# DassHydro-dev/smash

Measured on AMD Instinct MI355X. Metric: cell-timesteps/s, forward+adjoint sweep, higher is better.
Workload: dtype f32

## Files before the change

### __graft_entry__.py

```python
from __future__ import annotations

import os
import subprocess
import sys

ROOT = os.path.dirname(os.path.abspath(__file__))
if ROOT not in sys.path:
    sys.path.insert(0, ROOT)

HIPCC = os.environ.get("HIPCC", "/opt/rocm/bin/hipcc")
CSRC = os.path.join(ROOT, "smash_amd", "csrc")
LIB = os.path.join(ROOT, "smash_amd", "libsmashx.so")
LIB_EXACT = os.path.join(ROOT, "smash_amd", "libsmashx_exact.so")
HIP_FLAGS = ["-O3", "-ffp-contract=off", "--offload-arch=gfx950", "-fPIC", "-shared", "-std=c++17"]


def _newer(target, sources):
    if not os.path.exists(target):
        return False
    t = os.path.getmtime(target)
    return all(os.path.getmtime(s) <= t for s in sources)


def build() -> None:
    srcs = [os.path.join(CSRC, f) for f in sorted(os.listdir(CSRC)) if f.endswith((".hip", ".cpp", ".h"))]
    srcs += [os.path.join(ROOT, "include", "smashx.h"), os.path.join(ROOT, "include", "smashx_setup.h"),
             os.path.join(ROOT, "include", "smashx_forcing.h"), os.path.join(ROOT, "include", "smashx_prcp.h"),
             os.path.join(ROOT, "include", "smashx_signature.h"), os.path.join(ROOT, "include", "smashx_hyper.h"),
             os.path.join(ROOT, "include", "smashx_ann.h")]
    jobs = []
    for lib, extra in ((LIB, []), (LIB_EXACT, ["-DSX_EXACT_LIBM=1"])):
        if not _newer(lib, srcs):
            cmd = [HIPCC] + HIP_FLAGS + extra + ["-pthread", "-o", lib, os.path.join(CSRC, "smashx.hip"), os.path.join(CSRC, "sx_plan.cpp"),
                                                 os.path.join(CSRC, "sx_lbfgsb.cpp"), os.path.join(CSRC, "sx_hyper.cpp")]
            jobs.append((cmd, subprocess.Popen(cmd, cwd=ROOT)))
    for cmd, j in jobs:
        if j.wait() != 0:
            raise subprocess.CalledProcessError(j.returncode, cmd)
    subprocess.check_call(["make", "-s", "-C", os.path.join(ROOT, "oracle"), "liboracle.so", "liboracle64.so"])
    ref_src = os.environ.get("SMASH_REFERENCE", "/root/reference")
    ref_lib = os.path.join(ROOT, "oracle", "_ref", "libsmash_ref.so")
    dropin = os.path.join(ROOT, "oracle", "_ref", "libsmash_dropin.so")
    shim = [os.path.join(ROOT, "fortran", "smashx_dropin.f90"), os.path.join(ROOT, "fortran", "smashx_setulb.f90"),
            os.path.join(ROOT, "include", "smashx.h"), os.path.join(ROOT, "oracle", "ref", "ref_capi.f90"),
            os.path.join(ROOT, "oracle", "ref", "build_ref.sh")]
    native_lb = os.path.join(ROOT, "oracle", "_ref", "libsmash_dropin_lbfgsb.so")
    if os.path.isdir(os.path.join(ref_src, "smash", "solver")) and not (os.path.exists(ref_lib) and _newer(dropin, shim) and _newer(native_lb, shim)):
        subprocess.check_call(["bash", os.path.join(ROOT, "oracle", "ref", "build_ref.sh")])
    import smash_amd
    from smash_amd import _lib
    L = _lib.lib()
    missing = [s for s in _lib.SYMBOLS + _lib.SETUP_SYMBOLS + _lib.FORCING_SYMBOLS + _lib.PRCP_SYMBOLS + _lib.SIGNATURE_SYMBOLS + _lib.HYPER_DEVICE_SYMBOLS + _lib.ANN_SYMBOLS if not hasattr(L, s)]
    if missing:
        raise RuntimeError(f"libsmashx.so lacks {missing}")


def smoke() -> None:
    import numpy as np

    sys.path.insert(0, os.path.join(ROOT, "tests"))
    import golden_util as gu

    import smash_amd
    from oracle import pyoracle
    if not os.path.exists(LIB):
        build()
    g = gu.load("gr_b_16x16x96_nse_gaps")
    ref = pyoracle.run(g.structure, g.mesh, g.dt, g.prcp, g.pet, g.qobs, g.params, g.states, adjoint=True, **g.opts)
    for k, v in g.adj["parameters_b"].items():
        assert np.array_equal(ref["parameters_b"][k], v), k

    setup = smash_amd.SetupDT(0, g.mesh.ng, structure=g.structure, dt=g.dt, ntime_step=g.nt)
    setup.optimize.jobs_fun, setup.optimize.wjobs_fun = ["nse"], [1.0]
    mesh = smash_amd.MeshDT.from_synth(setup, g.mesh)
    inp = smash_amd.Input_DataDT(setup, mesh)
# ... 25 lines not shown
```

### include/smashx.h

```cpp
#ifndef SMASHX_H
#define SMASHX_H

#ifdef __cplusplus
extern "C" {
#endif

#define SMASHX_GNP 16
#define SMASHX_GNS 8

enum { SMASHX_GR_A = 1, SMASHX_GR_B = 2, SMASHX_GR_C = 3, SMASHX_GR_D = 4, SMASHX_VIC_A = 5 };
enum { SMASHX_NSE = 1, SMASHX_KGE = 2, SMASHX_KGE2 = 3, SMASHX_SE = 4, SMASHX_RMSE = 5, SMASHX_LOGARITHMIC = 6,
       SMASHX_CRC = 7, SMASHX_CFP2 = 8, SMASHX_CFP10 = 9, SMASHX_CFP50 = 10, SMASHX_CFP90 = 11, SMASHX_EPF = 12, SMASHX_ELT = 13,
       SMASHX_ERC = 14 };
enum { SMASHX_PRIOR = 1, SMASHX_SMOOTHING = 2, SMASHX_HARD_SMOOTHING = 3 };
enum { SMASHX_P_CI = 0, SMASHX_P_CP = 1, SMASHX_P_BETA = 2, SMASHX_P_CFT = 3, SMASHX_P_CST = 4, SMASHX_P_ALPHA = 5,
       SMASHX_P_EXC = 6, SMASHX_P_B = 7, SMASHX_P_CUSL1 = 8, SMASHX_P_CUSL2 = 9, SMASHX_P_CLSL = 10, SMASHX_P_KS = 11,
       SMASHX_P_DS = 12, SMASHX_P_DSM = 13, SMASHX_P_WS = 14, SMASHX_P_LR = 15 };
enum { SMASHX_S_HI = 0, SMASHX_S_HP = 1, SMASHX_S_HFT = 2, SMASHX_S_HST = 3, SMASHX_S_HUSL1 = 4, SMASHX_S_HUSL2 = 5,
       SMASHX_S_HLSL = 6, SMASHX_S_HLR = 7 };

enum {
    SMASHX_OK = 0,
    SMASHX_E_ARG = -1,
    SMASHX_E_UNSUPPORTED = -2,
// ... 186 lines not shown
};
int smashx_selftest_eval(int device, int fn, const float* x, const float* y, long long n, float* out0, float* out1);

#define SMASHX_LBFGSB_START 0
#define SMASHX_LBFGSB_FG 1
#define SMASHX_LBFGSB_NEW_X 2
#define SMASHX_LBFGSB_CONVERGED 3
#define SMASHX_LBFGSB_ABNORMAL 4
typedef struct smashx_lbfgsb smashx_lbfgsb;
int smashx_lbfgsb_create(long n, int m, const double* lower, const double* upper, double factr, double pgtol, smashx_lbfgsb** out);
int smashx_lbfgsb_step(smashx_lbfgsb* opt, double* x, double f, const double* g, int* task);
long smashx_lbfgsb_iterations(const smashx_lbfgsb* opt);
long smashx_lbfgsb_evaluations(const smashx_lbfgsb* opt);
double smashx_lbfgsb_projected_gradient(const smashx_lbfgsb* opt);
const char* smashx_lbfgsb_message(const smashx_lbfgsb* opt);
int smashx_lbfgsb_destroy(smashx_lbfgsb* opt);

#include "smashx_setup.h"
#include "smashx_forcing.h"
#include "smashx_prcp.h"
#include "smashx_signature.h"
#include "smashx_hyper.h"
#include "smashx_ann.h"

#ifdef __cplusplus
}
#endif
#endif
```

### smash_amd/_lib.py

```python
from __future__ import annotations

import ctypes as C
import os

_HERE = os.path.dirname(os.path.abspath(__file__))
EXACT = os.environ.get("SMASHX_EXACT_LIBM", "0") not in ("", "0")
LIB_PATH = os.environ.get("SMASHX_LIB", os.path.join(_HERE, "libsmashx_exact.so" if EXACT else "libsmashx.so"))

ABI_VERSION = 9
GNP, GNS = 16, 8
E_OK, E_ARG, E_UNSUPPORTED, E_HIP, E_NODEVICE, E_MESH, E_STATE = 0, -1, -2, -3, -4, -5, -6
STRUCTURES = {"gr-a": 1, "gr-b": 2, "gr-c": 3, "gr-d": 4, "vic-a": 5}
JOBS_FUN = {"nse": 1, "kge": 2, "kge2": 3, "se": 4, "rmse": 5, "logarithmic": 6,
            "Crc": 7, "Cfp2": 8, "Cfp10": 9, "Cfp50": 10, "Cfp90": 11, "Epf": 12, "Elt": 13, "Erc": 14}
SIGNATURE_FUN = ("Crc", "Cfp2", "Cfp10", "Cfp50", "Cfp90", "Epf", "Elt", "Erc")
JREG_FUN = {"prior": 1, "smoothing": 2, "hard_smoothing": 3}
HYPER = {"hyper-linear": 1, "hyper-polynomial": 2}
LBFGSB_START, LBFGSB_FG, LBFGSB_NEW_X, LBFGSB_CONVERGED, LBFGSB_ABNORMAL = range(5)
COMM_ID_BYTES = 128
FN = {k: i for i, k in enumerate("TANH TANH_BRANCHY EXPM1 EXP LOG POW POWB POW_M4 POW_M4_M5 POW_M025 POW_M025_M125 POW_3P5 POW_3P5_2P5 "
                                 "DIV DIV4 FDIV DIV_FAST".split())}
FN_COUNT = len(FN)

HALO_FN = C.CFUNCTYPE(C.c_int, C.c_void_p, C.c_int, C.c_int, C.c_int)
# ... 140 lines not shown
    "smashx_hyper_upload": (_int, [ptr, ptr, ptr]),
    "smashx_hyper_gradient": (_int, [ptr, ptr, ptr]),
    "smashx_hyper_fields": (_int, [ptr, _par, _sta]),
    "smashx_hyper_info": (_int, [ptr, ptr, ptr]),
}
HYPER_DEVICE_SYMBOLS = list(HYPER_DEVICE_PROTOTYPES)
ANN_LAYER = {"dense": 1, "relu": 2, "leaky_relu": 3, "elu": 4, "selu": 5, "sigmoid": 6, "tanh": 7, "scale": 8,
             "softplus": 9, "softmax": 10, "dropout": 11}
_graph = [_int, _int, ptr, ptr, _int]
ANN_PROTOTYPES = {
    "smashx_ann_set_descriptors": (_int, [ptr, _int, ptr]),
    "smashx_ann_set_net": (_int, [ptr, _int, ptr, ptr, _int, ptr, ptr, ptr]),
    "smashx_ann_upload": (_int, [ptr, ptr]),
    "smashx_ann_gradient": (_int, [ptr, ptr]),
    "smashx_ann_fields": (_int, [ptr, _par, _sta]),
    "smashx_ann_info": (_int, [ptr, ptr, ptr]),
    "smashx_ann_host_nweights": (_int, _graph),
    "smashx_ann_host_forward": (_int, _graph + [ptr, ptr, ptr, _long, ptr, ptr]),
    "smashx_ann_host_gradient": (_int, _graph + [ptr, ptr, ptr, _long, ptr, ptr, ptr]),
    "smashx_ann_host_activation": (_int, [_int, _long, ptr, ptr, ptr]),
    "smashx_ann_host_exp": (_int, [_long, ptr, ptr]),
}
ANN_SYMBOLS = list(ANN_PROTOTYPES)


class SmashxError(RuntimeError):
    def __init__(self, code, msg):
        super().__init__(f"libsmashx error {code}: {msg}")
        self.code = code


_lib = None


def lib():
    global _lib
    if _lib is None:
        if not os.path.exists(LIB_PATH):
            raise ImportError(f"{LIB_PATH} is missing: build the HIP library first (__graft_entry__.build()); "
                              "smash_amd has no CPU fallback")
        L = C.CDLL(LIB_PATH)
        for name, (restype, argtypes) in list(PROTOTYPES.items()) + list(SETUP_PROTOTYPES.items()) + list(FORCING_PROTOTYPES.items()) + list(PRCP_PROTOTYPES.items()) + list(SIGNATURE_PROTOTYPES.items()) + list(HYPER_DEVICE_PROTOTYPES.items()) + list(ANN_PROTOTYPES.items()):
            fn = getattr(L, name)
            fn.restype, fn.argtypes = restype, argtypes
        sizes = (C.c_int * 7)()
        L.smashx_abi_sizes(sizes)
        mine = [C.sizeof(t) for t in (Config, Mesh, Options, Parameters, States, Costs, Timing)]
        if list(sizes) != mine:
            raise ImportError(f"{LIB_PATH} was built from another include/smashx.h (struct sizes {list(sizes)}, this module expects {mine}): "
                              "rebuild it (__graft_entry__.build())")
        _lib = L
    return _lib


def check(rc):
    if rc != 0:
        raise SmashxError(rc, lib().smashx_last_error().decode())
```

### smash_amd/csrc/smashx.hip

```cpp
#include "../../include/smashx.h"

#include <hip/hip_runtime.h>
#include <rccl/rccl.h>

#include <dlfcn.h>

#include <algorithm>
#include <functional>
#include <numeric>
#include <cstdio>
#include <cstdlib>
#include <cstring>
#include <string>
#include <vector>

#include "sx_cost.h"
#include "sx_jreg.h"
#include "sx_kernels.h"
#include "sx_ensemble.h"
#include "sx_fields.h"
#include "sx_interception.h"
#include "sx_meanforcing.h"
#include "sx_prcpindices.h"
#include "sx_hypermap.h"
// ... 588 lines not shown
}

SxDeviceArrays view_at(const smashx_plan* p, int off) {
    SxDeviceArrays B = p->A;
    B.k0 = 0; B.k1 = p->n;
    const size_t q = (size_t)(off / 4);
    B.qtT = p->A.qtT + q * p->npad * 4;
    B.hrk = nullptr;
    if (p->A.hrT) { if (p->A.hr_skew) B.hr_row0 = (int)q; else B.hrT = p->A.hrT + q * p->npad * 4; }
    if (p->A.qdT) B.qdT = p->A.qdT + q * p->npad * 4;
    if (!p->chain) B.qsk = nullptr;
    B.xT = p->A.xT + q * p->A.nx * 4;
    if (p->A.qtdT) B.qtdT = p->A.qtdT + q * p->npad * 4;
    if (p->A.xdT) B.xdT = p->A.xdT + q * p->A.nx * 4;
    if (p->A.tape_hp) B.tape_hp = p->A.tape_hp + (size_t)off * p->npad;
    if (p->A.tape_hft) B.tape_hft = p->A.tape_hft + (size_t)off * p->npad;
    if (p->A.tape_hi) B.tape_hi = p->A.tape_hi + (size_t)off * p->npad;
    if (p->A.ckpt_hi) B.ckpt_hi = p->A.ckpt_hi + (size_t)(off / SX_HIK) * p->npad;
    if (p->A.tape_hst) B.tape_hst = p->A.tape_hst + (size_t)off * p->npad;
    return B;
}

typedef void (*VertKernel)(SxDeviceArrays, int, int);
VertKernel vert_fwd_kernel(int st, bool tape, bool compact) {
#define SX_GR(ST) {sx_k_vert_fwd<ST, false, false>, sx_k_vert_fwd<ST, false, true>, sx_k_vert_fwd<ST, true, false>, sx_k_vert_fwd<ST, true, true>}
    static const VertKernel k[5][4] = {SX_GR(1), SX_GR(2), SX_GR(3), SX_GR(4),
                                       {sx_k_vert_fwd_vic<false, false>, sx_k_vert_fwd_vic<false, true>, sx_k_vert_fwd_vic<true, false>, sx_k_vert_fwd_vic<true, true>}};
#undef SX_GR
    return k[st - 1][2 * tape + compact];
}
VertKernel vert_adj_kernel(int st, bool compact) {
    static const VertKernel k[5][2] = {{sx_k_vert_adj<1, false>, sx_k_vert_adj<1, true>}, {sx_k_vert_adj<2, false>, sx_k_vert_adj<2, true>},
                                       {sx_k_vert_adj<3, false>, sx_k_vert_adj<3, true>}, {sx_k_vert_adj<4, false>, sx_k_vert_adj<4, true>},
                                       {sx_k_vert_adj_vic<false>, sx_k_vert_adj_vic<true>}};
    return k[st - 1][compact];
}
VertKernel vert_tan_kernel(int st) {
    static const VertKernel k[5] = {sx_k_vert_fwd_d<1>, sx_k_vert_fwd_d<2>, sx_k_vert_fwd_d<3>, sx_k_vert_fwd_d<4>, sx_k_vert_fwd_vic_d};
    return k[st - 1];
}
void launch_vert(smashx_plan* p, VertKernel k, int kind, size_t lds, int off, int t0, int T) {
    const SxDeviceArrays B = view_at(p, off);
    if (B.k1 <= B.k0) return;
    const dim3 grid((B.k1 - B.k0 + SX_VBLOCK - 1) / SX_VBLOCK), block(SX_VBLOCK);
    p->mark_begin(kind, p->stream, (double)(B.k1 - B.k0) * T);
    hipLaunchKernelGGL(k, grid, block, lds, p->stream, B, t0, T);
    p->mark_end();
}
void vert_fwd(smashx_plan* p, int off, bool tape, int t0, int T) {
    launch_vert(p, vert_fwd_kernel(p->st, tape, p->A.prcp16 != nullptr), 0, p->st == 5 ? 0 : p->vlds_fwd, off, t0, T);
}
void vert_adj(smashx_plan* p, int off, int t0, int T) {
    launch_vert(p, vert_adj_kernel(p->st, p->A.prcp16 != nullptr), 3, p->st == 5 ? 0 : p->vlds_adj, off, t0, T);
}
void vert_tan(smashx_plan* p, int off, int t0, int T) { launch_vert(p, vert_tan_kernel(p->st), 0, 0, off, t0, T); }
double round_cells(const smashx_plan* p, int r0, int r1) {
    double c = 0.0;
    for (int r = r0; r < r1; ++r) c += p->round_ncells[r];
    return c;
}
int chain_first(const smashx_plan* p) {
    const int nr = p->sch.nrounds;
    return (p->chain && nr - p->chain_from >= 2) ? p->chain_from : nr;
}
void reset_chain_counters(smashx_plan* p, hipStream_t st) {
    (void)hipMemsetAsync(p->A.prog, 0, (size_t)p->sch.ngroups * sizeof(int), st);
    (void)hipMemsetAsync(p->A.prog + p->sch.ngroups + 1, 0, sizeof(int), st);
}
void route_fwd_rounds(smashx_plan* p, int off, bool tape, int t0, int T, hipStream_t st, int r0, int r1, int tan = 0) {
    SxDeviceArrays B = view_at(p, off);
    if (!p->dom_q_active) B.qdT = nullptr;
    if (tan) B.qsk = nullptr;
    const size_t lds = (size_t)2 * p->M * sizeof(float4);
    void (*const k)(SxDeviceArrays, int, int, int, int) = tan == 1 ? sx_k_route_fwd<true, false, 1> : tan == 2 ? sx_k_route_fwd<false, false, 2>
                                                         : tape ? sx_k_route_fwd<true, false> : sx_k_route_fwd<false, false>;
    for (int r = r0; r < r1; ++r) {
// ... 1351 lines not shown

int smashx_halo_edges(const smashx_plan* p, int* out_src, int* out_dst, int* in_src, int* in_dst) {
    if (!p) return fail(SMASHX_E_ARG, "null plan");
    for (int i = 0; i < p->n_out; ++i) { if (out_src) out_src[i] = p->sch.out_src[i]; if (out_dst) out_dst[i] = p->sch.out_dst[i]; }
    for (int i = 0; i < p->n_in; ++i) { if (in_src) in_src[i] = p->sch.in_src[i]; if (in_dst) in_dst[i] = p->sch.in_dst[i]; }
    return 0;
}

int smashx_plan_chunking(smashx_plan* p, int* chunk_steps, int* pipe_steps) {
    if (!p) return fail(SMASHX_E_ARG, "null plan");
    int rc = set_device(p); if (rc) return rc;
    if ((rc = ensure_chunk_buffers(p, true))) return rc;
    if (chunk_steps) *chunk_steps = p->Tc;
    if (pipe_steps) *pipe_steps = p->Tp;
    return 0;
}

int smashx_plan_hbm(const smashx_plan* p, double out[3]) {
    if (!p || !out) return fail(SMASHX_E_ARG, "null argument");
    out[0] = p->hbm_free_at_plan; out[1] = p->hbm_total; out[2] = p->bytes;
    return 0;
}

int smashx_set_halo(smashx_plan* p, float* d_out_buf, float* d_in_buf, smashx_halo_fn fn, void* user) {
    if (!p) return fail(SMASHX_E_ARG, "null plan");
    if (fn && ((p->n_out > 0 && !d_out_buf) || (p->n_in > 0 && !d_in_buf))) return fail(SMASHX_E_ARG, "halo buffers missing");
    p->halo_out = d_out_buf; p->halo_in = d_in_buf; p->halo_fn = fn; p->halo_user = user;
    return 0;
}

int smashx_set_median_slots(smashx_plan* p, int nslots, const int* slot_of_gauge, smashx_reduce_fn fn, void* user) {
    if (!p || nslots < 0 || (nslots > 0 && !slot_of_gauge)) return fail(SMASHX_E_ARG, "bad argument");
    int rc = set_device(p); if (rc) return rc;
    p->med_nslots = 0; p->med_fn = fn; p->med_user = user;
    if (nslots == 0) return 0;
    std::vector<int> sl(std::max(p->ng, 1), -1);
    for (int g = 0; g < p->ng; ++g) {
        sl[g] = slot_of_gauge[g];
        if (sl[g] < -1 || sl[g] >= nslots) return fail(SMASHX_E_ARG, "slot_of_gauge out of range");
    }
    if (p->d_med_slot) { p->dfree(p->d_med_slot); p->dfree(p->d_medx); p->dfree(p->d_medx_idx); }
    if ((rc = p->upload_vec(&p->d_med_slot, sl))) return rc;
    p->med_slot_h = sl;
    if ((rc = p->dmalloc(&p->d_medx, (size_t)3 * nslots))) return rc;
    if ((rc = p->dmalloc(&p->d_medx_idx, (size_t)nslots))) return rc;
    p->med_nslots = nslots;
// ... 1325 lines not shown
```

### smash_amd/csrc/sx_kernels.h

```cpp
#pragma once

#include <hip/hip_runtime.h>

#include <climits>

#include "sx_ops.h"
#include "sx_tangent.h"
#include "sx_vic.h"

#define SX_BT 4
#define SX_VBLOCK 256

__device__ __forceinline__ void sx_lds_barrier() {
    __builtin_amdgcn_fence(__ATOMIC_RELEASE, "workgroup", "local");
    __builtin_amdgcn_s_barrier();
    __builtin_amdgcn_fence(__ATOMIC_ACQUIRE, "workgroup", "local");
}

__device__ __forceinline__ void sx_lds_wave_fence() {
    __builtin_amdgcn_fence(__ATOMIC_RELEASE, "workgroup", "local");
    __builtin_amdgcn_wave_barrier();
    __builtin_amdgcn_fence(__ATOMIC_ACQUIRE, "workgroup", "local");
}

// ... 35 lines not shown
}
__device__ __forceinline__ void sx_gstore4(float4* p, const float4& q) {
#if defined(__HIP_DEVICE_COMPILE__)
    sx_f4v v; v.x = q.x; v.y = q.y; v.z = q.z; v.w = q.w;
    *(__attribute__((address_space(1))) sx_f4v*)p = v;
#else
    *p = q;
#endif
}
__device__ __forceinline__ float sx_gload1(const float* p) {
#if defined(__HIP_DEVICE_COMPILE__)
    return *(const __attribute__((address_space(1))) float*)p;
#else
    return *p;
#endif
}

__device__ __forceinline__ void sx_pin(float4& v) {
    asm volatile("" : "+v"(v.x), "+v"(v.y), "+v"(v.z), "+v"(v.w) : : "memory");
}

__device__ __forceinline__ void sx_pin1(float& v) { asm volatile("" : "+v"(v) : : "memory"); }
__device__ __forceinline__ void sx_pinu(unsigned& v) { asm volatile("" : "+v"(v) : : "memory"); }

typedef __attribute__((address_space(1))) int sx_gint;
#define SX_PROG_STALL(A) ((A).prog + (A).ngroups)
#define SX_PROG_TICKET(A) ((A).prog + (A).ngroups + 1)
#define SX_PROG_EXTRA 8
#ifndef SX_PK
#define SX_PK 16
#endif
#define SX_SPIN_LIMIT (1 << 22)
__device__ __forceinline__ void sx_wait_prog(const int* prog, int need, int& seen, int* stalled, int limit, int tag = -1) {
    if (seen >= need) return;
    int spins = 0;
    while (seen < need) {
        seen = __hip_atomic_load((const sx_gint*)prog, __ATOMIC_RELAXED, __HIP_MEMORY_SCOPE_AGENT);
        if (seen < need) {
            const bool out = ++spins > limit;
            if (out || (spins & 1023) == 0) {
                if (out) {
                    if (atomicCAS(stalled + 3, 0, tag + 2) == 0) { stalled[4] = (int)(prog - stalled); stalled[5] = need; stalled[6] = seen; }
                    __hip_atomic_store((sx_gint*)stalled, 1, __ATOMIC_RELAXED, __HIP_MEMORY_SCOPE_AGENT);
                }
                if (out || __hip_atomic_load((const sx_gint*)stalled, __ATOMIC_RELAXED, __HIP_MEMORY_SCOPE_AGENT)) { seen = 0x7fffffff; break; }
            }
// ... 136 lines not shown
    typedef int sx_v4i __attribute__((ext_vector_type(4)));
    const __amdgpu_buffer_rsrc_t r = __builtin_amdgcn_make_buffer_rsrc((void*)row, 0, 0x7fffffff, 0x00020000);
    sx_v4i v = {__builtin_bit_cast(int, a), __builtin_bit_cast(int, b), __builtin_bit_cast(int, c), __builtin_bit_cast(int, d)};
    __builtin_amdgcn_raw_buffer_store_b128(v, r, byte_off, 0, AUX);
}
template <int AUX = 0>
__device__ __forceinline__ void sx_row_store(float* row, unsigned byte_off, float v) {
    const __amdgpu_buffer_rsrc_t r = __builtin_amdgcn_make_buffer_rsrc((void*)row, 0, 0x7fffffff, 0x00020000);
    __builtin_amdgcn_raw_buffer_store_b32(__builtin_bit_cast(int, v), r, byte_off, 0, AUX);
}

template <int AUX = 0>
__device__ __forceinline__ unsigned sx_row_load_u16(const unsigned short* row, unsigned byte_off) {
    const __amdgpu_buffer_rsrc_t r = __builtin_amdgcn_make_buffer_rsrc((void*)row, 0, 0x7fffffff, 0x00020000);
    return (unsigned)(unsigned short)__builtin_amdgcn_raw_buffer_load_b16(r, byte_off, 0, AUX);
}

__device__ __forceinline__ float sx_prcp_decode(const SxDeviceArrays& A, unsigned k) {
    const float v = (float)k * A.prcp_c;
    return k == 65535u ? A.prcp_gap : v;
}

typedef const __attribute__((address_space(4))) float sx_cfloat;
template <bool COMPACT>
struct SxForcing {
    const SxDeviceArrays& A;
    const unsigned kb;
    const size_t npad;
    int h;
    const char* prow; const char* erow;
    unsigned p_n, p_w; float e_n, e_w, r_n, r_w;
    __device__ __forceinline__ SxForcing(const SxDeviceArrays& A_, unsigned kb_, int t_first)
        : A(A_), kb(kb_), npad((size_t)A_.npad), h(COMPACT ? (t_first + A_.hour0) % 24 : 0),
          prow(COMPACT ? (const char*)(A_.prcp16 + (size_t)t_first * A_.npad) : (const char*)(A_.prcp + (size_t)t_first * A_.npad)),
          erow(COMPACT ? nullptr : (const char*)(A_.pet + (size_t)t_first * A_.npad)),
          p_n(0u), p_w(0u), e_n(0.f), e_w(0.f), r_n(0.f), r_w(0.f) {}
    template <int AUX, bool BACK> __device__ __forceinline__ void request(int t, bool first) {
        const long step = (long)npad * (COMPACT ? 2 : 4) * (BACK ? -1 : 1);
        if (!COMPACT) {
            p_n = __float_as_uint(sx_row_load<AUX>((const float*)prow, kb));
            e_n = sx_row_load<AUX>((const float*)erow, kb);
            prow += step; erow += step;
            return;
        }
        p_n = __float_as_uint(sx_row_load<AUX>((const float*)prow, (kb >> 1) & ~3u));
        prow += step;
        if (first || h == (BACK ? 23 : 0)) e_n = sx_row_load<AUX>(A.petd + (size_t)((t + A.hour0) / 24) * npad, kb);
        r_n = sx_row_load(A.pet_ratio + h, 0u);
        h = BACK ? (h == 0 ? 23 : h - 1) : (h == 23 ? 0 : h + 1);
    }
    __device__ __forceinline__ void hold() {
        p_w = p_n; e_w = e_n; r_w = r_n;
        sx_pinu(p_w); sx_pin1(e_w);
        if (COMPACT) sx_pin1(r_w);
    }
    __device__ __forceinline__ float prcp() const {
        if (!COMPACT) return __uint_as_float(p_w);
        return sx_prcp_decode(A, (p_w >> ((kb & 4u) << 2)) & 0xffffu);
    }
    __device__ __forceinline__ float pet() const {
        if (!COMPACT) return e_w;
        return e_w < 0.f ? e_w : e_w * r_w;
    }
};

__device__ __forceinline__ void sx_forcing_at(const SxDeviceArrays& A, int t, unsigned kb, float& p, float& e) {
    const size_t npad = (size_t)A.npad;
    if (A.prcp16 == nullptr) { p = sx_row_load(A.prcp + (size_t)t * npad, kb); e = sx_row_load(A.pet + (size_t)t * npad, kb); return; }
    p = sx_prcp_decode(A, sx_row_load_u16(A.prcp16 + (size_t)t * npad, kb >> 1));
    const int q = t + A.hour0;
    const float D = sx_row_load(A.petd + (size_t)(q / 24) * npad, kb);
    e = D < 0.f ? D : D * ((sx_cfloat*)A.pet_ratio)[q % 24];
}

#ifndef SX_VFWD_WAVES
#define SX_VFWD_WAVES 8
#endif
template <int ST, bool TAPE, bool CF>
#ifndef SX_VFWD_WAVES_GRC
#define SX_VFWD_WAVES_GRC 7
#endif
__global__ __launch_bounds__(SX_VBLOCK, (ST == 2 && CF) ? SX_VFWD_WAVES : (ST == 3 && TAPE && CF) ? SX_VFWD_WAVES_GRC : 1)
void sx_k_vert_fwd(SxDeviceArrays A, int t0, int T) {
    SX_LIBM_INIT();
    const int k = A.k0 + blockIdx.x * SX_VBLOCK + threadIdx.x;
    if (k >= A.k1) return;
    const size_t npad = (size_t)A.npad;

    SxCellParams P;
    float hi = 0.f, hp = 0.f, hft = 0.f, hst = 0.f;
    P.ci = (ST == 2 || ST == 3) ? A.ci[k] : 1.f;
    P.cp = A.cp[k];
    P.cft = A.cft[k];
    P.cst = (ST == 3) ? A.cst[k] : 1.f;
    P.exc = (ST != 4) ? A.exc[k] : 0.f;
    sx_cell_params_init(P);
    P.cft_m4 = sx_pow_m4(P.cft);
    P.cst_m4 = (ST == 3) ? sx_pow_m4(P.cst) : 1.f;
    if (ST == 2 || ST == 3) hi = A.hi[k];
    hp = A.hp[k];
    hft = A.hft[k];
    if (ST == 3) hst = A.hst[k];

    const unsigned kb = (unsigned)k * 4u;
    SxForcing<CF> F(A, kb, t0);
    if (T > 0) F.template request<SX_NT, false>(t0, true);
    for (int tq = 0; tq * 4 < T; ++tq) {
        float q[4] = {0.f, 0.f, 0.f, 0.f};
#pragma unroll
        for (int i = 0; i < 4; ++i) {
            const int tt = tq * 4 + i;
            if (tt < T) {
                F.hold();
                if (tt + 1 < T) F.template request<SX_NT, false>(t0 + tt + 1, false);
                const float prcp = F.prcp(), pet = F.pet();
                if (TAPE) {
                    const size_t o = (size_t)tt * npad;
                    if (ST == 2 || ST == 3) {
                        if (A.tape_hi) sx_row_store<SX_NT>(A.tape_hi + o, kb, hi);
                        else if ((tt % SX_HIK) == 0) sx_row_store<SX_NT>(A.ckpt_hi + (size_t)(tt / SX_HIK) * npad, kb, hi);
                    }
                    sx_row_store<SX_NT>(A.tape_hp + o, kb, hp);
                    sx_row_store<SX_NT>(A.tape_hft + o, kb, hft);
                    if (ST == 3) sx_row_store<SX_NT>(A.tape_hst + o, kb, hst);
                }
                const bool still = SX_STILL && sx_wave_all(sx_is_still<ST>(prcp, pet, hi, hp));
                q[i] = sx_vertical_step<ST>(P, prcp, pet, hi, hp, hft, hst, still);
            }
        }
        sx_row_store4<SX_NT>(A.qtT + (size_t)tq * npad * 4, kb * 4u, q[0], q[1], q[2], q[3]);
    }
    if (ST == 2 || ST == 3) A.hi[k] = hi;
    A.hp[k] = hp;
    A.hft[k] = hft;
    if (ST == 3) A.hst[k] = hst;
}

__device__ __forceinline__ SxVicParams sx_vic_load(const SxDeviceArrays& A, int k) {
    SxVicParams P;
    P.b = A.ci[k]; P.cusl1 = A.cp[k]; P.cusl2 = A.cft[k]; P.clsl = A.cst[k]; P.ks = A.exc[k];
    P.ds = A.px[0][k]; P.dsm = A.px[1][k]; P.ws = A.px[2][k];
    sx_vic_derive(P);
    return P;
}
#ifndef SX_VFWD_WAVES_VIC
#define SX_VFWD_WAVES_VIC 5
#endif
template <bool TAPE, bool CF>
__global__ __launch_bounds__(SX_VBLOCK, TAPE ? SX_VFWD_WAVES_VIC : 1) void sx_k_vert_fwd_vic(SxDeviceArrays A, int t0, int T) {
    SX_LIBM_INIT();
    const int k = A.k0 + blockIdx.x * SX_VBLOCK + threadIdx.x;
    if (k >= A.k1) return;
    const size_t npad = (size_t)A.npad;
// ... 562 lines not shown
    if (valid && cell >= 0) { A.hlr_b[cell] = hr_b; A.lr_b[cell] = lr_b; }
    if (A.gtime && j == 0) A.gtime[2 * (A.ngroups + g) + 1] = wall_clock64();
    if (CHAIN) {
        asm volatile("s_waitcnt vmcnt(0)" ::: "memory");
        __builtin_amdgcn_s_barrier();
        if (j == 0 && g != A.mute_group) sx_publish(A.prog + g, nb);
    }
}

template <bool CHAIN>
__global__ __launch_bounds__(SX_MAXGROUP, SX_RLB_A) void sx_k_route_adj(SxDeviceArrays A, int g0, int gend, int t0, int T) {
    if (SX_R_PRIO) __builtin_amdgcn_s_setprio(SX_R_PRIO);
    if (!CHAIN) { sx_route_adj_group<false>(A, g0 + (int)blockIdx.x, g0, gend, t0, T); return; }
    for (;;) {
        const int ticket = sx_next_ticket(A);
        if (ticket >= gend - g0) break;
        sx_route_adj_group<CHAIN>(A, gend - 1 - ticket, g0, gend, t0, T);
    }
}

#ifndef SX_VADJ_WAVES
#define SX_VADJ_WAVES 5
#endif
template <int ST, bool CF>
#ifndef SX_VADJ_WAVES_GRC
#if SX_EXACT_LIBM
#define SX_VADJ_WAVES_GRC 1
#else
#define SX_VADJ_WAVES_GRC 5
#endif
#endif
__global__ __launch_bounds__(SX_VBLOCK, (ST == 2 && CF) ? SX_VADJ_WAVES : (ST == 3 && CF) ? SX_VADJ_WAVES_GRC : 1)
void sx_k_vert_adj(SxDeviceArrays A, int t0, int T) {
    SX_LIBM_INIT();
    const int k = A.k0 + blockIdx.x * SX_VBLOCK + threadIdx.x;
    if (k >= A.k1) return;
    const size_t npad = (size_t)A.npad;
    SxCellParams P;
    P.ci = (ST == 2 || ST == 3) ? A.ci[k] : 1.f;
    P.cp = A.cp[k];
    P.cft = A.cft[k];
    P.cst = (ST == 3) ? A.cst[k] : 1.f;
    P.exc = (ST != 4) ? A.exc[k] : 0.f;
    sx_cell_params_init(P);
    SxAdjParams Q;
    Q.cst_m5 = 1.f;
    sx_pow_m4_m5(P.cft, &P.cft_m4, &Q.cft_m5);
    P.cst_m4 = 1.f;
    if (ST == 3) sx_pow_m4_m5(P.cst, &P.cst_m4, &Q.cst_m5);
    Q.dcft2 = sx_mkdiv(P.cft * P.cft);
    Q.dcst2 = sx_mkdiv(P.cst * P.cst);
    Q.dcp2 = sx_mkdiv(P.cp * P.cp);
    SxCellGrads G;
    G.ci_b = (ST == 2 || ST == 3) ? A.ci_b[k] : 0.f;
    G.cp_b = A.cp_b[k];
    G.cft_b = A.cft_b[k];
    G.cst_b = (ST == 3) ? A.cst_b[k] : 0.f;
    G.exc_b = (ST != 4) ? A.exc_b[k] : 0.f;
    G.hi_b = (ST == 2 || ST == 3) ? A.hi_b[k] : 0.f;
    G.hp_b = A.hp_b[k];
    G.hft_b = A.hft_b[k];
    G.hst_b = (ST == 3) ? A.hst_b[k] : 0.f;
    const unsigned kb = (unsigned)k * 4u;
    SxForcing<CF> F(A, kb, t0 + T - 1);
    float n_hi = 0.f, n_hp = 0.f, n_hft = 0.f, n_hst = 0.f, n_q = 0.f;
    const bool hi_taped = (ST == 2 || ST == 3) && A.tape_hi != nullptr;
    const size_t olast = (size_t)(T > 0 ? T - 1 : 0) * npad;
    const float* r_hi = hi_taped ? A.tape_hi + olast : nullptr;
    const float* r_hp = A.tape_hp + olast;
    const float* r_hft = A.tape_hft + olast;
    const float* r_hst = (ST == 3) ? A.tape_hst + olast : nullptr;
    auto fetch = [&](int tt, bool first) {
        F.template request<SX_VADJ_NT, true>(t0 + tt, first);
        if (hi_taped) { n_hi = sx_row_load<SX_VADJ_NT>(r_hi, kb); r_hi -= npad; }
        n_hp = sx_row_load<SX_VADJ_NT>(r_hp, kb); n_hft = sx_row_load<SX_VADJ_NT>(r_hft, kb);
        r_hp -= npad; r_hft -= npad;
        if (ST == 3) { n_hst = sx_row_load<SX_VADJ_NT>(r_hst, kb); r_hst -= npad; }
        n_q = sx_row_load(A.qtT + (size_t)(tt >> 2) * npad * 4 + (tt & 3), kb * 4u);
    };
    __shared__ float s_hi[(ST == 2 || ST == 3) ? SX_HIK : 1][SX_VBLOCK];
    if (T > 0) fetch(T - 1, true);
    for (int tb = (T - 1) / SX_HIK; tb >= 0; --tb) {
        const int tt0 = tb * SX_HIK, len = min(SX_HIK, T - tt0);
        if ((ST == 2 || ST == 3) && !hi_taped) {
            float fp[SX_HIK], fe[SX_HIK];
#pragma unroll
            for (int j = 0; j < SX_HIK; ++j) sx_forcing_at(A, t0 + tt0 + (j < len ? j : 0), kb, fp[j], fe[j]);
            float h = sx_row_load(A.ckpt_hi + (size_t)tb * npad, kb);
#pragma unroll
            for (int j = 0; j < SX_HIK; ++j) {
                s_hi[j][threadIdx.x] = h;
                if (j < len && fp[j] >= 0.f && fe[j] >= 0.f) { float pn, ei; sx_interception(fp[j], fe[j], P.ci, P.dci, h, pn, ei); }
            }
        }
        for (int tt = tt0 + len - 1; tt >= tt0; --tt) {
            float hit = n_hi, hp = n_hp, hft = n_hft, hst = n_hst, q = n_q;
            F.hold();
            sx_pin1(hp); sx_pin1(hft); sx_pin1(q);
            if (ST == 2 || ST == 3) sx_pin1(hit);
            if (ST == 3) sx_pin1(hst);
            if (tt > 0) fetch(tt - 1, false);
            const float prcp = F.prcp(), pet = F.pet();
            const float hi = (ST == 2 || ST == 3) ? (hi_taped ? hit : s_hi[tt - tt0][threadIdx.x]) : 0.f;
            const bool still = SX_STILL && sx_wave_all(sx_is_still<ST>(prcp, pet, hi, hp));
            sx_vertical_step_b<ST>(P, Q, prcp, pet, hi, hp, hft, hst, q, G, still);
        }
    }
    if (ST == 2 || ST == 3) { A.ci_b[k] = G.ci_b; A.hi_b[k] = G.hi_b; }
    A.cp_b[k] = G.cp_b;
    A.cft_b[k] = G.cft_b;
    if (ST == 3) { A.cst_b[k] = G.cst_b; A.hst_b[k] = G.hst_b; }
    if (ST != 4) A.exc_b[k] = G.exc_b;
    A.hp_b[k] = G.hp_b;
    A.hft_b[k] = G.hft_b;
}
```

### smash_amd/solver.py

```python
from __future__ import annotations

import ctypes as C

import zlib

import numpy as np

from . import _lib
from ._lib import HYPER, JOBS_FUN, JREG_FUN, SIGNATURE_FUN, STRUCTURES
from .synth import PARAM_DEFAULTS, PARAM_NAMES, STATE_NAMES


RATIO_PET_HOURLY = np.array([0, 0, 0, 0, 0, 0, 0, 0.035, 0.062, 0.079, 0.097, 0.11, 0.117, 0.117, 0.11, 0.097, 0.079, 0.062, 0.035,
                             0, 0, 0, 0, 0], dtype=np.float32)


def _ptr(a):
    return a.ctypes.data_as(C.c_void_p) if a is not None else None


def make_config(setup, mesh, chunk_steps=0, pipe_steps=0, group_size=0, device=-1, tile=None):
    cfg = _lib.Config()
    cfg.structure, cfg.nrow, cfg.ncol = STRUCTURES[setup.structure], mesh.nrow, mesh.ncol
    cfg.nt, cfg.ng, cfg.dt, cfg.dx = setup.ntime_step, mesh.ng, setup.dt, mesh.dx
# ... 296 lines not shown
        return x

    def control_gradient(self):
        g = np.zeros(self.control_size(), np.float64)
        _lib.check(_lib.lib().smashx_control_gradient(self._h, _ptr(g)))
        return g

    def cost_and_qsim(self, output):
        qs = np.zeros((self.ng, self.nt), np.float32, order="F") if self.ng else None
        costs = _lib.Costs()
        _lib.check(_lib.lib().smashx_download(self._h, 0, None, None, _ptr(qs), C.byref(costs), None, None, None))
        return _store_costs(output, qs, costs)

    def sweep(self, adjoint=False, cost_b=1.0):
        _lib.check(_lib.lib().smashx_sweep(self._h, bool(adjoint), cost_b))

    def timing(self):
        t = _lib.Timing()
        _lib.check(_lib.lib().smashx_get_timing(self._h, C.byref(t)))
        d = {k: getattr(t, k) for k, _ in _lib.Timing._fields_ if k != "cellsteps"}
        for i, k in enumerate(("vert_fwd", "route_fwd", "route_adj", "vert_adj")):
            d[k + "_cellsteps"] = float(t.cellsteps[i])
        return d

    def download(self, adjoint, parameters, states, output, parameters_b=None, states_b=None, only_b=None):
        P, k1 = _pack(parameters, PARAM_NAMES, _lib.Parameters)
        S, k2 = _pack(states, STATE_NAMES, _lib.States)
        qs = np.zeros((self.ng, self.nt), np.float32, order="F") if self.ng else None
        costs = _lib.Costs()
        F = PB = SB = None
        kf = kp = ks = None
        if not adjoint and output is not None:
            F, kf = _pack(output.fstates, STATE_NAMES, _lib.States)
        if adjoint:
            PB, kp = _pack(parameters_b, PARAM_NAMES, _lib.Parameters, only_b)
            SB, ks = _pack(states_b, STATE_NAMES, _lib.States, only_b)
        _lib.check(_lib.lib().smashx_download(self._h, bool(adjoint), C.byref(P), C.byref(S), _ptr(qs), C.byref(costs),
                                              C.byref(F) if F is not None else None,
                                              C.byref(PB) if PB is not None else None,
                                              C.byref(SB) if SB is not None else None))
        return _store_costs(output, qs, costs)

    def multiple_run(self, parameters, states, sample, ind_parameters_states, return_qsim=False, *, res_cost=None, res_qsim=None):
        sample, ind = check_multiple_run(self.structure, self.ng, self.nt, sample, ind_parameters_states, res_cost, res_qsim)
        nf, S = sample.shape
        if res_cost is None:
# ... 591 lines not shown
```

Measured before the change: 57.66 billion.

## Template vertical kernels on hi-tape mode and add multi-step forcing prefetch ring

Makes whether the interception level is taped a compile-time template parameter of the forward and adjoint vertical kernels, so each variant drops the runtime branch and gets its own launch bounds. Both kernels gain a depth-D register ring that prefetches forcing and tape values several steps ahead, using asm moves to keep the loads from being reordered. The prefetch depths SX_VPF_F and SX_VPF_A default to 1, so by default the main gains are the specialised kernels and restructured loops. A query function exposing the hi-tape mode is also added.

```diff
diff --git a/__graft_entry__.py b/__graft_entry__.py
--- a/__graft_entry__.py
+++ b/__graft_entry__.py
@@ -27,7 +27,7 @@
     srcs += [os.path.join(ROOT, "include", "smashx.h"), os.path.join(ROOT, "include", "smashx_setup.h"),
              os.path.join(ROOT, "include", "smashx_forcing.h"), os.path.join(ROOT, "include", "smashx_prcp.h"),
              os.path.join(ROOT, "include", "smashx_signature.h"), os.path.join(ROOT, "include", "smashx_hyper.h"),
-             os.path.join(ROOT, "include", "smashx_ann.h")]
+             os.path.join(ROOT, "include", "smashx_ann.h"), os.path.join(ROOT, "include", "smashx_vertical.h")]
     jobs = []
     for lib, extra in ((LIB, []), (LIB_EXACT, ["-DSX_EXACT_LIBM=1"])):
         if not _newer(lib, srcs):
@@ -50,7 +50,7 @@
     import smash_amd
     from smash_amd import _lib
     L = _lib.lib()
-    missing = [s for s in _lib.SYMBOLS + _lib.SETUP_SYMBOLS + _lib.FORCING_SYMBOLS + _lib.PRCP_SYMBOLS + _lib.SIGNATURE_SYMBOLS + _lib.HYPER_DEVICE_SYMBOLS + _lib.ANN_SYMBOLS if not hasattr(L, s)]
+    missing = [s for s in _lib.SYMBOLS + _lib.SETUP_SYMBOLS + _lib.FORCING_SYMBOLS + _lib.PRCP_SYMBOLS + _lib.SIGNATURE_SYMBOLS + _lib.HYPER_DEVICE_SYMBOLS + _lib.ANN_SYMBOLS + _lib.VERTICAL_SYMBOLS if not hasattr(L, s)]
     if missing:
         raise RuntimeError(f"libsmashx.so lacks {missing}")
 
diff --git a/include/smashx.h b/include/smashx.h
--- a/include/smashx.h
+++ b/include/smashx.h
@@ -232,6 +232,7 @@
 #include "smashx_signature.h"
 #include "smashx_hyper.h"
 #include "smashx_ann.h"
+#include "smashx_vertical.h"
 
 #ifdef __cplusplus
 }
diff --git a/include/smashx_vertical.h b/include/smashx_vertical.h
--- /dev/null
+++ b/include/smashx_vertical.h
@@ -0,0 +1,15 @@
+#ifndef SMASHX_VERTICAL_H
+#define SMASHX_VERTICAL_H
+
+#include "smashx.h"
+
+#ifdef __cplusplus
+extern "C" {
+#endif
+
+int smashx_plan_hi_tape(const smashx_plan* plan, int* hi_tape);
+
+#ifdef __cplusplus
+}
+#endif
+#endif
diff --git a/smash_amd/_lib.py b/smash_amd/_lib.py
--- a/smash_amd/_lib.py
+++ b/smash_amd/_lib.py
@@ -186,6 +186,10 @@
     "smashx_ann_host_exp": (_int, [_long, ptr, ptr]),
 }
 ANN_SYMBOLS = list(ANN_PROTOTYPES)
+VERTICAL_PROTOTYPES = {
+    "smashx_plan_hi_tape": (_int, [ptr, ptr]),
+}
+VERTICAL_SYMBOLS = list(VERTICAL_PROTOTYPES)
 
 
 class SmashxError(RuntimeError):
@@ -204,7 +208,7 @@
             raise ImportError(f"{LIB_PATH} is missing: build the HIP library first (__graft_entry__.build()); "
                               "smash_amd has no CPU fallback")
         L = C.CDLL(LIB_PATH)
-        for name, (restype, argtypes) in list(PROTOTYPES.items()) + list(SETUP_PROTOTYPES.items()) + list(FORCING_PROTOTYPES.items()) + list(PRCP_PROTOTYPES.items()) + list(SIGNATURE_PROTOTYPES.items()) + list(HYPER_DEVICE_PROTOTYPES.items()) + list(ANN_PROTOTYPES.items()):
+        for name, (restype, argtypes) in list(PROTOTYPES.items()) + list(SETUP_PROTOTYPES.items()) + list(FORCING_PROTOTYPES.items()) + list(PRCP_PROTOTYPES.items()) + list(SIGNATURE_PROTOTYPES.items()) + list(HYPER_DEVICE_PROTOTYPES.items()) + list(ANN_PROTOTYPES.items()) + list(VERTICAL_PROTOTYPES.items()):
             fn = getattr(L, name)
             fn.restype, fn.argtypes = restype, argtypes
         sizes = (C.c_int * 7)()
diff --git a/smash_amd/csrc/smashx.hip b/smash_amd/csrc/smashx.hip
--- a/smash_amd/csrc/smashx.hip
+++ b/smash_amd/csrc/smashx.hip
@@ -634,18 +634,23 @@
 }
 
 typedef void (*VertKernel)(SxDeviceArrays, int, int);
-VertKernel vert_fwd_kernel(int st, bool tape, bool compact) {
-#define SX_GR(ST) {sx_k_vert_fwd<ST, false, false>, sx_k_vert_fwd<ST, false, true>, sx_k_vert_fwd<ST, true, false>, sx_k_vert_fwd<ST, true, true>}
-    static const VertKernel k[5][4] = {SX_GR(1), SX_GR(2), SX_GR(3), SX_GR(4),
-                                       {sx_k_vert_fwd_vic<false, false>, sx_k_vert_fwd_vic<false, true>, sx_k_vert_fwd_vic<true, false>, sx_k_vert_fwd_vic<true, true>}};
+VertKernel vert_fwd_kernel(int st, bool tape, bool compact, bool hi_taped) {
+#define SX_GR(ST, HI) {sx_k_vert_fwd<ST, false, false>, sx_k_vert_fwd<ST, false, true>, sx_k_vert_fwd<ST, true, false, HI>, sx_k_vert_fwd<ST, true, true, HI>}
+    static const VertKernel k[2][5][4] = {
+        {SX_GR(1, true), SX_GR(2, false), SX_GR(3, false), SX_GR(4, true),
+         {sx_k_vert_fwd_vic<false, false>, sx_k_vert_fwd_vic<false, true>, sx_k_vert_fwd_vic<true, false>, sx_k_vert_fwd_vic<true, true>}},
+        {SX_GR(1, true), SX_GR(2, true), SX_GR(3, true), SX_GR(4, true),
+         {sx_k_vert_fwd_vic<false, false>, sx_k_vert_fwd_vic<false, true>, sx_k_vert_fwd_vic<true, false>, sx_k_vert_fwd_vic<true, true>}}};
 #undef SX_GR
-    return k[st - 1][2 * tape + compact];
-}
-VertKernel vert_adj_kernel(int st, bool compact) {
-    static const VertKernel k[5][2] = {{sx_k_vert_adj<1, false>, sx_k_vert_adj<1, true>}, {sx_k_vert_adj<2, false>, sx_k_vert_adj<2, true>},
-                                       {sx_k_vert_adj<3, false>, sx_k_vert_adj<3, true>}, {sx_k_vert_adj<4, false>, sx_k_vert_adj<4, true>},
-                                       {sx_k_vert_adj_vic<false>, sx_k_vert_adj_vic<true>}};
-    return k[st - 1][compact];
+    return k[hi_taped][st - 1][2 * tape + compact];
+}
+VertKernel vert_adj_kernel(int st, bool compact, bool hi_taped) {
+#define SX_GR(ST, HI) {sx_k_vert_adj<ST, false, HI>, sx_k_vert_adj<ST, true, HI>}
+    static const VertKernel k[2][5][2] = {
+        {SX_GR(1, true), SX_GR(2, false), SX_GR(3, false), SX_GR(4, true), {sx_k_vert_adj_vic<false>, sx_k_vert_adj_vic<true>}},
+        {SX_GR(1, true), SX_GR(2, true), SX_GR(3, true), SX_GR(4, true), {sx_k_vert_adj_vic<false>, sx_k_vert_adj_vic<true>}}};
+#undef SX_GR
+    return k[hi_taped][st - 1][compact];
 }
 VertKernel vert_tan_kernel(int st) {
     static const VertKernel k[5] = {sx_k_vert_fwd_d<1>, sx_k_vert_fwd_d<2>, sx_k_vert_fwd_d<3>, sx_k_vert_fwd_d<4>, sx_k_vert_fwd_vic_d};
@@ -660,10 +665,10 @@
     p->mark_end();
 }
 void vert_fwd(smashx_plan* p, int off, bool tape, int t0, int T) {
-    launch_vert(p, vert_fwd_kernel(p->st, tape, p->A.prcp16 != nullptr), 0, p->st == 5 ? 0 : p->vlds_fwd, off, t0, T);
+    launch_vert(p, vert_fwd_kernel(p->st, tape, p->A.prcp16 != nullptr, p->hi_tape), 0, p->st == 5 ? 0 : p->vlds_fwd, off, t0, T);
 }
 void vert_adj(smashx_plan* p, int off, int t0, int T) {
-    launch_vert(p, vert_adj_kernel(p->st, p->A.prcp16 != nullptr), 3, p->st == 5 ? 0 : p->vlds_adj, off, t0, T);
+    launch_vert(p, vert_adj_kernel(p->st, p->A.prcp16 != nullptr, p->hi_tape), 3, p->st == 5 ? 0 : p->vlds_adj, off, t0, T);
 }
 void vert_tan(smashx_plan* p, int off, int t0, int T) { launch_vert(p, vert_tan_kernel(p->st), 0, 0, off, t0, T); }
 double round_cells(const smashx_plan* p, int r0, int r1) {
@@ -2061,6 +2066,12 @@
     return 0;
 }
 
+int smashx_plan_hi_tape(const smashx_plan* p, int* hi_tape) {
+    if (!p || !hi_tape) return fail(SMASHX_E_ARG, "null argument");
+    *hi_tape = p->chunk_ready ? (p->hi_tape ? 1 : 0) : -1;
+    return 0;
+}
+
 int smashx_set_halo(smashx_plan* p, float* d_out_buf, float* d_in_buf, smashx_halo_fn fn, void* user) {
     if (!p) return fail(SMASHX_E_ARG, "null plan");
     if (fn && ((p->n_out > 0 && !d_out_buf) || (p->n_in > 0 && !d_in_buf))) return fail(SMASHX_E_ARG, "halo buffers missing");
diff --git a/smash_amd/csrc/sx_kernels.h b/smash_amd/csrc/sx_kernels.h
--- a/smash_amd/csrc/sx_kernels.h
+++ b/smash_amd/csrc/sx_kernels.h
@@ -81,6 +81,8 @@
 
 __device__ __forceinline__ void sx_pin1(float& v) { asm volatile("" : "+v"(v) : : "memory"); }
 __device__ __forceinline__ void sx_pinu(unsigned& v) { asm volatile("" : "+v"(v) : : "memory"); }
+__device__ __forceinline__ float sx_take(const float& slot) { float v; asm volatile("v_mov_b32 %0, %1" : "=v"(v) : "v"(slot) : "memory"); return v; }
+__device__ __forceinline__ unsigned sx_takeu(const unsigned& slot) { unsigned v; asm volatile("v_mov_b32 %0, %1" : "=v"(v) : "v"(slot) : "memory"); return v; }
 
 typedef __attribute__((address_space(1))) int sx_gint;
 #define SX_PROG_STALL(A) ((A).prog + (A).ngroups)
@@ -263,37 +265,50 @@
 }
 
 typedef const __attribute__((address_space(4))) float sx_cfloat;
-template <bool COMPACT>
+template <bool COMPACT, int D = 1>
 struct SxForcing {
+    static_assert(D >= 1 && D <= 24, "at most one day boundary inside the ring");
     const SxDeviceArrays& A;
     const unsigned kb;
     const size_t npad;
     int h;
+    int hh;
     const char* prow; const char* erow;
-    unsigned p_n, p_w; float e_n, e_w, r_n, r_w;
+    unsigned p_n[D], p_w; float e_n[D], e_w, r_n[D], r_w;
     __device__ __forceinline__ SxForcing(const SxDeviceArrays& A_, unsigned kb_, int t_first)
-        : A(A_), kb(kb_), npad((size_t)A_.npad), h(COMPACT ? (t_first + A_.hour0) % 24 : 0),
+        : A(A_), kb(kb_), npad((size_t)A_.npad), h(COMPACT ? (t_first + A_.hour0) % 24 : 0), hh(h),
           prow(COMPACT ? (const char*)(A_.prcp16 + (size_t)t_first * A_.npad) : (const char*)(A_.prcp + (size_t)t_first * A_.npad)),
           erow(COMPACT ? nullptr : (const char*)(A_.pet + (size_t)t_first * A_.npad)),
-          p_n(0u), p_w(0u), e_n(0.f), e_w(0.f), r_n(0.f), r_w(0.f) {}
-    template <int AUX, bool BACK> __device__ __forceinline__ void request(int t, bool first) {
+          p_w(0u), e_w(0.f), r_w(0.f) {
+#pragma unroll
+        for (int j = 0; j < D; ++j) { p_n[j] = 0u; e_n[j] = 0.f; r_n[j] = 0.f; }
+    }
+    template <int AUX, bool BACK> __device__ __forceinline__ void request(int t, bool first, int J = 0) {
         const long step = (long)npad * (COMPACT ? 2 : 4) * (BACK ? -1 : 1);
         if (!COMPACT) {
-            p_n = __float_as_uint(sx_row_load<AUX>((const float*)prow, kb));
-            e_n = sx_row_load<AUX>((const float*)erow, kb);
+            p_n[J] = __float_as_uint(sx_row_load<AUX>((const float*)prow, kb));
+            e_n[J] = sx_row_load<AUX>((const float*)erow, kb);
             prow += step; erow += step;
             return;
         }
-        p_n = __float_as_uint(sx_row_load<AUX>((const float*)prow, (kb >> 1) & ~3u));
+        p_n[J] = __float_as_uint(sx_row_load<AUX>((const float*)prow, (kb >> 1) & ~3u));
         prow += step;
-        if (first || h == (BACK ? 23 : 0)) e_n = sx_row_load<AUX>(A.petd + (size_t)((t + A.hour0) / 24) * npad, kb);
-        r_n = sx_row_load(A.pet_ratio + h, 0u);
+        if (first || h == (BACK ? 23 : 0)) e_n[J] = sx_row_load<AUX>(A.petd + (size_t)((t + A.hour0) / 24) * npad, kb);
+        r_n[J] = sx_row_load(A.pet_ratio + h, 0u);
         h = BACK ? (h == 0 ? 23 : h - 1) : (h == 23 ? 0 : h + 1);
     }
-    __device__ __forceinline__ void hold() {
-        p_w = p_n; e_w = e_n; r_w = r_n;
-        sx_pinu(p_w); sx_pin1(e_w);
-        if (COMPACT) sx_pin1(r_w);
+    template <bool BACK = false> __device__ __forceinline__ void hold(bool first = false, int J = 0) {
+        if (D == 1) {
+            p_w = p_n[0]; e_w = e_n[0]; r_w = r_n[0];
+            sx_pinu(p_w); sx_pin1(e_w);
+            if (COMPACT) sx_pin1(r_w);
+            return;
+        }
+        p_w = sx_takeu(p_n[J]);
+        if (!COMPACT) { e_w = sx_take(e_n[J]); return; }
+        if (first || hh == (BACK ? 23 : 0)) e_w = sx_take(e_n[J]);
+        r_w = sx_take(r_n[J]);
+        hh = BACK ? (hh == 0 ? 23 : hh - 1) : (hh == 23 ? 0 : hh + 1);
     }
     __device__ __forceinline__ float prcp() const {
         if (!COMPACT) return __uint_as_float(p_w);
@@ -317,7 +332,10 @@
 #ifndef SX_VFWD_WAVES
 #define SX_VFWD_WAVES 8
 #endif
-template <int ST, bool TAPE, bool CF>
+#ifndef SX_VPF_F
+#define SX_VPF_F 1
+#endif
+template <int ST, bool TAPE, bool CF, bool HI_TAPED = true>
 #ifndef SX_VFWD_WAVES_GRC
 #define SX_VFWD_WAVES_GRC 7
 #endif
@@ -344,21 +362,22 @@
     if (ST == 3) hst = A.hst[k];
 
     const unsigned kb = (unsigned)k * 4u;
-    SxForcing<CF> F(A, kb, t0);
-    if (T > 0) F.template request<SX_NT, false>(t0, true);
-    for (int tq = 0; tq * 4 < T; ++tq) {
+    constexpr int D = (ST == 3) ? 1 : SX_VPF_F;
+    constexpr int U = (D == 3) ? 12 : 4;
+    SxForcing<CF, D> F(A, kb, t0);
+    auto quad = [&](int tt4, int j0, bool guard) __attribute__((always_inline)) {
         float q[4] = {0.f, 0.f, 0.f, 0.f};
 #pragma unroll
         for (int i = 0; i < 4; ++i) {
-            const int tt = tq * 4 + i;
-            if (tt < T) {
-                F.hold();
-                if (tt + 1 < T) F.template request<SX_NT, false>(t0 + tt + 1, false);
+            const int tt = tt4 + i, J = (j0 + i) % D;
+            if (!guard || tt < T) {
+                F.template hold<false>(tt == 0, J);
+                if (!guard || tt + D < T) F.template request<SX_NT, false>(t0 + tt + D, false, J);
                 const float prcp = F.prcp(), pet = F.pet();
                 if (TAPE) {
                     const size_t o = (size_t)tt * npad;
                     if (ST == 2 || ST == 3) {
-                        if (A.tape_hi) sx_row_store<SX_NT>(A.tape_hi + o, kb, hi);
+                        if (HI_TAPED) sx_row_store<SX_NT>(A.tape_hi + o, kb, hi);
                         else if ((tt % SX_HIK) == 0) sx_row_store<SX_NT>(A.ckpt_hi + (size_t)(tt / SX_HIK) * npad, kb, hi);
                     }
                     sx_row_store<SX_NT>(A.tape_hp + o, kb, hp);
@@ -369,7 +388,25 @@
                 q[i] = sx_vertical_step<ST>(P, prcp, pet, hi, hp, hft, hst, still);
             }
         }
-        sx_row_store4<SX_NT>(A.qtT + (size_t)tq * npad * 4, kb * 4u, q[0], q[1], q[2], q[3]);
+        sx_row_store4<SX_NT>(A.qtT + (size_t)(tt4 >> 2) * npad * 4, kb * 4u, q[0], q[1], q[2], q[3]);
+    };
+    int tu = 0;
+    if (D > 1 && U + D <= T) {
+#pragma unroll
+        for (int j = 0; j < D; ++j) F.template request<SX_NT, false>(t0 + j, j == 0, j);
+        for (; tu + U + D <= T; tu += U) {
+#pragma unroll
+            for (int g = 0; g < U / 4; ++g) quad(tu + 4 * g, (4 * g) % D, false);
+        }
+    } else {
+#pragma unroll
+        for (int j = 0; j < D; ++j)
+            if (j < T) F.template request<SX_NT, false>(t0 + j, j == 0, j);
+    }
+    for (; tu < T; tu += U) {
+#pragma unroll
+        for (int g = 0; g < U / 4; ++g)
+            if (tu + 4 * g < T) quad(tu + 4 * g, (4 * g) % D, true);
     }
     if (ST == 2 || ST == 3) A.hi[k] = hi;
     A.hp[k] = hp;
@@ -978,7 +1015,11 @@
 #ifndef SX_VADJ_WAVES
 #define SX_VADJ_WAVES 5
 #endif
-template <int ST, bool CF>
+#define SX_VADJ_WAVES_LEAN 5
+#ifndef SX_VPF_A
+#define SX_VPF_A 1
+#endif
+template <int ST, bool CF, bool HI_TAPED>
 #ifndef SX_VADJ_WAVES_GRC
 #if SX_EXACT_LIBM
 #define SX_VADJ_WAVES_GRC 1
@@ -986,7 +1027,7 @@
 #define SX_VADJ_WAVES_GRC 5
 #endif
 #endif
-__global__ __launch_bounds__(SX_VBLOCK, (ST == 2 && CF) ? SX_VADJ_WAVES : (ST == 3 && CF) ? SX_VADJ_WAVES_GRC : 1)
+__global__ __launch_bounds__(SX_VBLOCK, (ST == 2 && CF) ? (HI_TAPED ? SX_VADJ_WAVES : SX_VADJ_WAVES_LEAN) : (ST == 3 && CF) ? SX_VADJ_WAVES_GRC : 1)
 void sx_k_vert_adj(SxDeviceArrays A, int t0, int T) {
     SX_LIBM_INIT();
     const int k = A.k0 + blockIdx.x * SX_VBLOCK + threadIdx.x;
@@ -1018,27 +1059,69 @@
     G.hft_b = A.hft_b[k];
     G.hst_b = (ST == 3) ? A.hst_b[k] : 0.f;
     const unsigned kb = (unsigned)k * 4u;
-    SxForcing<CF> F(A, kb, t0 + T - 1);
-    float n_hi = 0.f, n_hp = 0.f, n_hft = 0.f, n_hst = 0.f, n_q = 0.f;
-    const bool hi_taped = (ST == 2 || ST == 3) && A.tape_hi != nullptr;
+    static_assert(HI_TAPED || ST == 2 || ST == 3, "only gr-b / gr-c have an interception level to rebuild");
+    constexpr bool HAS_HI = (ST == 2 || ST == 3);
+    constexpr int D = (ST == 3 || !HI_TAPED) ? 1 : SX_VPF_A;
+    SxForcing<CF, D> F(A, kb, t0 + T - 1);
+    float n_hi[D], n_hp[D], n_hft[D], n_hst[D], n_q[D];
+#pragma unroll
+    for (int j = 0; j < D; ++j) n_hi[j] = n_hp[j] = n_hft[j] = n_hst[j] = n_q[j] = 0.f;
     const size_t olast = (size_t)(T > 0 ? T - 1 : 0) * npad;
-    const float* r_hi = hi_taped ? A.tape_hi + olast : nullptr;
+    const float* r_hi = (HAS_HI && HI_TAPED) ? A.tape_hi + olast : nullptr;
     const float* r_hp = A.tape_hp + olast;
     const float* r_hft = A.tape_hft + olast;
     const float* r_hst = (ST == 3) ? A.tape_hst + olast : nullptr;
-    auto fetch = [&](int tt, bool first) {
-        F.template request<SX_VADJ_NT, true>(t0 + tt, first);
-        if (hi_taped) { n_hi = sx_row_load<SX_VADJ_NT>(r_hi, kb); r_hi -= npad; }
-        n_hp = sx_row_load<SX_VADJ_NT>(r_hp, kb); n_hft = sx_row_load<SX_VADJ_NT>(r_hft, kb);
+    auto fetch = [&](int tt, bool first, int J) __attribute__((always_inline)) {
+        F.template request<SX_VADJ_NT, true>(t0 + tt, first, J);
+        if (HAS_HI && HI_TAPED) { n_hi[J] = sx_row_load<SX_VADJ_NT>(r_hi, kb); r_hi -= npad; }
+        n_hp[J] = sx_row_load<SX_VADJ_NT>(r_hp, kb); n_hft[J] = sx_row_load<SX_VADJ_NT>(r_hft, kb);
         r_hp -= npad; r_hft -= npad;
-        if (ST == 3) { n_hst = sx_row_load<SX_VADJ_NT>(r_hst, kb); r_hst -= npad; }
-        n_q = sx_row_load(A.qtT + (size_t)(tt >> 2) * npad * 4 + (tt & 3), kb * 4u);
+        if (ST == 3) { n_hst[J] = sx_row_load<SX_VADJ_NT>(r_hst, kb); r_hst -= npad; }
+        n_q[J] = sx_row_load(A.qtT + (size_t)(tt >> 2) * npad * 4 + (tt & 3), kb * 4u);
     };
-    __shared__ float s_hi[(ST == 2 || ST == 3) ? SX_HIK : 1][SX_VBLOCK];
-    if (T > 0) fetch(T - 1, true);
-    for (int tb = (T - 1) / SX_HIK; tb >= 0; --tb) {
-        const int tt0 = tb * SX_HIK, len = min(SX_HIK, T - tt0);
-        if ((ST == 2 || ST == 3) && !hi_taped) {
+    auto step = [&](int tt, int J, bool guard, float hi_rebuilt) __attribute__((always_inline)) {
+        float hit = 0.f, hp, hft, hst = 0.f, q;
+        F.template hold<true>(tt == T - 1, J);
+        if (D == 1) {
+            hit = n_hi[0]; hp = n_hp[0]; hft = n_hft[0]; hst = n_hst[0]; q = n_q[0];
+            sx_pin1(hp); sx_pin1(hft); sx_pin1(q);
+            if (HAS_HI && HI_TAPED) sx_pin1(hit);
+            if (ST == 3) sx_pin1(hst);
+        } else {
+            if (HAS_HI && HI_TAPED) hit = sx_take(n_hi[J]);
+            hp = sx_take(n_hp[J]); hft = sx_take(n_hft[J]);
+            if (ST == 3) hst = sx_take(n_hst[J]);
+            q = sx_take(n_q[J]);
+        }
+        if (!guard || tt - D >= 0) fetch(tt - D, false, J);
+        const float prcp = F.prcp(), pet = F.pet();
+        const float hi = HAS_HI ? (HI_TAPED ? hit : hi_rebuilt) : 0.f;
+        const bool still = SX_STILL && sx_wave_all(sx_is_still<ST>(prcp, pet, hi, hp));
+        sx_vertical_step_b<ST>(P, Q, prcp, pet, hi, hp, hft, hst, q, G, still);
+    };
+    int tt = T - 1;
+    if (D > 1 && T >= 2 * D) {
+#pragma unroll
+        for (int j = 0; j < D; ++j) fetch(T - 1 - j, j == 0, j);
+        for (; tt - (2 * D - 1) >= 0; tt -= D) {
+#pragma unroll
+            for (int j = 0; j < D; ++j) step(tt - j, j, false, 0.f);
+        }
+    } else {
+#pragma unroll
+        for (int j = 0; j < D; ++j)
+            if (T - 1 - j >= 0) fetch(T - 1 - j, j == 0, j);
+    }
+    if constexpr (HI_TAPED) {
+        for (; tt >= 0; tt -= D) {
+#pragma unroll
+            for (int j = 0; j < D; ++j)
+                if (tt - j >= 0) step(tt - j, j, true, 0.f);
+        }
+    } else {
+        __shared__ float s_hi[SX_HIK][SX_VBLOCK];
+        for (int tb = (T - 1) / SX_HIK; tb >= 0; --tb) {
+            const int tt0 = tb * SX_HIK, len = min(SX_HIK, T - tt0);
             float fp[SX_HIK], fe[SX_HIK];
 #pragma unroll
             for (int j = 0; j < SX_HIK; ++j) sx_forcing_at(A, t0 + tt0 + (j < len ? j : 0), kb, fp[j], fe[j]);
@@ -1048,18 +1131,7 @@
                 s_hi[j][threadIdx.x] = h;
                 if (j < len && fp[j] >= 0.f && fe[j] >= 0.f) { float pn, ei; sx_interception(fp[j], fe[j], P.ci, P.dci, h, pn, ei); }
             }
-        }
-        for (int tt = tt0 + len - 1; tt >= tt0; --tt) {
-            float hit = n_hi, hp = n_hp, hft = n_hft, hst = n_hst, q = n_q;
-            F.hold();
-            sx_pin1(hp); sx_pin1(hft); sx_pin1(q);
-            if (ST == 2 || ST == 3) sx_pin1(hit);
-            if (ST == 3) sx_pin1(hst);
-            if (tt > 0) fetch(tt - 1, false);
-            const float prcp = F.prcp(), pet = F.pet();
-            const float hi = (ST == 2 || ST == 3) ? (hi_taped ? hit : s_hi[tt - tt0][threadIdx.x]) : 0.f;
-            const bool still = SX_STILL && sx_wave_all(sx_is_still<ST>(prcp, pet, hi, hp));
-            sx_vertical_step_b<ST>(P, Q, prcp, pet, hi, hp, hft, hst, q, G, still);
+            for (int tt = tt0 + len - 1; tt >= tt0; --tt) step(tt, 0, true, s_hi[tt - tt0][threadIdx.x]);
         }
     }
     if (ST == 2 || ST == 3) { A.ci_b[k] = G.ci_b; A.hi_b[k] = G.hi_b; }
diff --git a/smash_amd/solver.py b/smash_amd/solver.py
--- a/smash_amd/solver.py
+++ b/smash_amd/solver.py
@@ -342,6 +342,11 @@
         for i, k in enumerate(("vert_fwd", "route_fwd", "route_adj", "vert_adj")):
             d[k + "_cellsteps"] = float(t.cellsteps[i])
         return d
+
+    def hi_tape(self):
+        v = C.c_int(-1)
+        _lib.check(_lib.lib().smashx_plan_hi_tape(self._h, C.byref(v)))
+        return v.value
 
     def download(self, adjoint, parameters, states, output, parameters_b=None, states_b=None, only_b=None):
         P, k1 = _pack(parameters, PARAM_NAMES, _lib.Parameters)
```

Result: no change. 57.63 billion (-0.0%).
